# songxf1024/GIMS

Measured on NVIDIA B200. Metric: image_pairs_per_sec_2048kp, higher is better.
Workload: dtype f32

## Files before the change

gims_b200/csrc/gemm_tc.cu:

```cuda
#include "common.cuh"
#include "tc_common.cuh"

namespace gims {

namespace tc {

EncodeTiledFn get_encode_tiled() {
  static EncodeTiledFn fn = nullptr;
  if (fn) return fn;
  void* p = nullptr;
  cudaDriverEntryPointQueryResult qres;
  if (cudaGetDriverEntryPoint("cuTensorMapEncodeTiled", &p, cudaEnableDefault, &qres) != cudaSuccess ||
      qres != cudaDriverEntryPointSuccess)
    return nullptr;
  fn = reinterpret_cast<EncodeTiledFn>(p);
  return fn;
}

int make_tmap_f32_k32(CUtensorMap* out, const float* base, uint64_t rows, uint64_t cols, uint64_t ld, uint32_t box_rows) {
  EncodeTiledFn enc = get_encode_tiled();
  if (!enc) { set_error("cuTensorMapEncodeTiled entry point not available"); return GIMS_ERR_CUDA; }
  cuuint64_t dims[2] = {cols, rows};
  cuuint64_t strides[1] = {ld * sizeof(float)};
  cuuint32_t box[2] = {32, box_rows};
// ... 24 lines not shown
              (unsigned long long)rows, (unsigned long long)cols, (unsigned long long)ld, box_rows);
    return GIMS_ERR_CUDA;
  }
  return GIMS_OK;
}

}

namespace {

using namespace tc;

constexpr int BM = 128, BK = 32;
constexpr int kThreadsTc = 224;
__host__ __device__ constexpr int tc_threads(int prec) { return prec ? kThreadsTc + 128 : kThreadsTc; }

template <int BN, int PREC>
struct TcCfg {
  static constexpr int kBlockK = PREC ? 64 : 32;
  static constexpr int kABytes = BM * kBlockK * 4;
  static constexpr int kWBytes = PREC ? BN * 64 * 2 : BN * BK * 4;
  static constexpr int kStageBytes = kABytes + 2 * kWBytes;
  static constexpr int kStages = PREC ? (BN <= 64 ? 2 : (BN <= 128 ? 3 : 2))
                                      : ((BN <= 64) ? 3 : (BN <= 128 ? 4 : 3));
  static constexpr int kIssuers = 2;
  static constexpr bool kFold = true;
  static constexpr int kMainAcc = 2;
  static constexpr int kCorrAcc = kFold ? 0 : kIssuers;
  static constexpr int kAccCols = (kMainAcc + kCorrAcc) * BN;
  static constexpr int kTmemCols = (BN <= 64) ? 256 : 512;
  static constexpr int kRing = (kTmemCols - kAccCols) / 64 >= 4 ? 4 : 2;
  static constexpr int kRingCol = kAccCols;
  static_assert(kAccCols + kRing * 64 <= kTmemCols, "accumulators + A ring exceed TMEM");
  static constexpr int kBarriers = 2 * kStages + 2 * kRing + 1;
  static constexpr int kBiasOff = (kBarriers * 8 + 16 + 15) & ~15;
  static constexpr int kSmemBytes = kStages * kStageBytes + 1024  + kBiasOff + BN * 4;
};

struct TcArgs {
  int K0, K1;
  const float* bias;
  const float* R; int ldr;
  float* Y; int ldy;
  int N;
  int relu;
  float scale;
  int score;
  Segs segs;
  int tile_end[kMaxSegs];
  int qkv;
  float* qp; void* kp; void* vt; int ldv; int rows_total; int vbase[kMaxSegs];
  unsigned* status;
  const float* wscale_inv;
  int single_chain;
};

__device__ long long* g_gemm_trace = nullptr;

struct TileCoord { int seg, rows, ncols, r0, c0, rbase; };

template <int BN, int MODE, int PREC, typename Ready>
__device__ __forceinline__ void epilogue_tile(const TcArgs& g, const TileCoord& tcd, uint32_t lane_base, int n_main, int n_corr,
                                              int grp, int kGroups, int q, int lane, uint32_t stg, const float* bias_s,
                                              Ready&& ready, long long* trace, bool tr0) {
  using Cfg = TcCfg<BN, PREC>;
  const int seg = tcd.seg, rows = tcd.rows, ncols = tcd.ncols, r0 = tcd.r0, c0 = tcd.c0, rbase = tcd.rbase;
  const float wsc = (PREC && g.wscale_inv) ? *g.wscale_inv : 1.f;
  constexpr int kStgLd = 36;
  const int rl0 = lane >> 3, cj = (lane & 7) * 4;
  const int rfirst = r0 + 32 * q + rl0;
  const int nvalid = rows - rfirst;
  const bool use_r = MODE == 0 && g.R != nullptr;
  const float* rrow = use_r ? g.R + (size_t)(rbase + rfirst) * g.ldr + c0 + cj : nullptr;
  float4 rres[8];
#pragma unroll
  for (int i = 0; i < 8; ++i)
    rres[i] = (use_r && 4 * i < nvalid && c0 + 32 * grp + cj < ncols) ? *reinterpret_cast<const float4*>(rrow + (size_t)(4 * i) * g.ldr + 32 * grp)
                                                           : make_float4(0.f, 0.f, 0.f, 0.f);
  ready();
  if (trace && tr0) trace[3] = clock64();
#pragma unroll 1
  for (int cc = grp; cc < BN / 32; cc += kGroups) {
    uint32_t v[32];
    const uint32_t lane_col = lane_base + (uint32_t)(cc * 32);
    tmem_ld_32x32(lane_col, v);
    tmem_ld_wait();
    for (int a = 1; a < Cfg::kMainAcc + Cfg::kCorrAcc; ++a) {
      if (a < Cfg::kMainAcc ? a >= n_main : a - Cfg::kMainAcc >= n_corr) continue;
      uint32_t w[32];
      tmem_ld_32x32(lane_col + (uint32_t)(a * BN), w);
      tmem_ld_wait();
#pragma unroll
      for (int j = 0; j < 32; ++j) v[j] = __float_as_uint(__uint_as_float(v[j]) + __uint_as_float(w[j]));
    }
    if (PREC) {
#pragma unroll
      for (int j = 0; j < 32; ++j) v[j] = __float_as_uint(__uint_as_float(v[j]) * wsc);
    }
    if (trace && tr0 && cc < 2) trace[56 + 3 * cc] = clock64();
    const int c = c0 + cc * 32;
    if (c >= ncols) continue;
    if (MODE >= 2 && c >= 2 * kD) {
      const int r = r0 + 32 * q + lane;
      if (r < ((g.segs.nmax[seg] + 63) & ~63)) {
        const bool row_ok = r < rows;
        const int cc256 = c & 255;
        const size_t kcol = (size_t)g.vbase[seg] + r;
// ... 291 lines not shown
            hi[j] = __float_as_uint(h); x[j] = __float_as_uint(l);
          }
        }
        mbar_wait(&tfree[slot], ((uint32_t)(kb / Cfg::kRing) & 1u) ^ 1u);
        tcgen05_fence_after();
        if (trace && tr0 && kb < 8) trace[48 + kb] = clock64();
        if (PREC) {
          uint32_t h16[16], l16[16];
#pragma unroll
          for (int j = 0; j < 16; ++j) { h16[j] = hi[j]; l16[j] = x[j]; }
          tmem_st_32x16(lane_base + Cfg::kRingCol + slot * 64 + 16 * grp, h16);
          tmem_st_32x16(lane_base + Cfg::kRingCol + slot * 64 + 32 + 16 * grp, l16);
        } else {
          tmem_st_32x32(lane_base + Cfg::kRingCol + slot * 64, hi);
          tmem_st_32x32(lane_base + Cfg::kRingCol + slot * 64 + 32, x);
        }
        tmem_st_wait();
        tcgen05_fence_before();
        __syncwarp();
        if (lane == 0) mbar_arrive(&conv[slot]);
        if (trace && tr0 && kb < 8) trace[16 + kb] = clock64();
        if (++s == Cfg::kStages) { s = 0; ph ^= 1; }
      }
    }
    if (PREC && g.status && amax >= 32768.f && r0 + t < rows) atomicOr(g.status, GIMS_STATUS_FP16_RANGE);
    {
      const int n_main = nkb < Cfg::kMainAcc ? nkb : Cfg::kMainAcc;
      const int n_corr = nkb < Cfg::kCorrAcc ? nkb : Cfg::kCorrAcc;
      const TileCoord tcd = {seg, rows, ncols, r0, c0, rbase};
      const uint32_t stg = smem_u32(smem) + (uint32_t)((q + 4 * grp) * 32 * 36 * 4);
      epilogue_tile<BN, MODE, PREC>(g, tcd, lane_base, n_main, n_corr, grp, kGroups, q, lane, stg, bias_s,
                                    [&] { mbar_wait(accum_full, 0); tcgen05_fence_after(); }, trace, tr0);
    }
    tcgen05_fence_before();
    if (trace && tr0) trace[4] = clock64();
  }
  __syncthreads();
  if (warp == kWarpMma) {
    tcgen05_fence_after();
    tmem_dealloc<Cfg::kTmemCols>(tmem_base);
  }
  if (trace && threadIdx.x == 0) {
    trace[5] = clock64();
    unsigned long long gt; asm volatile("mov.u64 %0, %%globaltimer;" : "=l"(gt));
    trace[7] = (long long)gt;
  }
}

constexpr int kThreadsP = 480;
struct TcpCfg {
  static constexpr int BN = 128;
  static constexpr int kBlockK = 64;
  static constexpr int kABytes = BM * kBlockK * 4;
  static constexpr int kWBytes = BN * 64 * 2;
  static constexpr int kStageBytes = kABytes + 2 * kWBytes;
  static constexpr int kStages = 3;
  static constexpr int kRing = 2;
  static constexpr int kParkCol = 2 * BN;
  static constexpr int kRingCol = 3 * BN;
  static constexpr int kStgBytes = 4 * 32 * 36 * 4;
  static constexpr int kBarriers = 2 * kStages + 2 * kRing + 4;
  static constexpr int kBiasOff = (kBarriers * 8 + 16 + 15) & ~15;
  static constexpr int kSmemBytes = kStages * kStageBytes + kStgBytes + 1024  + kBiasOff + 2 * BN * 4;
};

template <int MODE, int PLANES>
__global__ void __launch_bounds__(kThreadsP, 1)
k_gemm_tcp(const __grid_constant__ CUtensorMap mapA0, const __grid_constant__ CUtensorMap mapA1,
           const __grid_constant__ CUtensorMap mapWhi, const __grid_constant__ CUtensorMap mapWlo, TcArgs g, int col_tiles,
           int total_work) {
  using Cfg = TcpCfg;
  constexpr int BN = Cfg::BN;
  extern __shared__ uint8_t smem_raw[];
  uint8_t* smem = reinterpret_cast<uint8_t*>((reinterpret_cast<uintptr_t>(smem_raw) + 1023) & ~uintptr_t(1023));
  uint8_t* stg_base = smem + Cfg::kStages * Cfg::kStageBytes;
  uint64_t* bars = reinterpret_cast<uint64_t*>(stg_base + Cfg::kStgBytes);
  uint64_t* full = bars;
  uint64_t* empty = bars + Cfg::kStages;
  uint64_t* conv = bars + 2 * Cfg::kStages;
  uint64_t* tfree = conv + Cfg::kRing;
  uint64_t* accum_full = tfree + Cfg::kRing;
  uint64_t* acc_free = accum_full + 1;
  uint64_t* park_full = acc_free + 1;
  uint64_t* park_free = park_full + 1;
  uint32_t* tmem_slot = reinterpret_cast<uint32_t*>(park_free + 1);
  float* bias_s = reinterpret_cast<float*>(reinterpret_cast<uint8_t*>(bars) + Cfg::kBiasOff);

  const int warp = threadIdx.x >> 5, lane = threadIdx.x & 31;
  constexpr int kWarpTma = 4, kWarpMma = 5, kWarpEpi = 11;
  long long* trace = (blockIdx.x == 0 && lane == 0) ? g_gemm_trace : nullptr;
  if (trace && threadIdx.x == 0) trace[0] = clock64();
#define TCP_TRACE(k) do { if (trace && lt < 4) trace[8 + lt * 8 + (k)] = clock64(); } while (0)
  const int nkb = (g.K0 + g.K1) / Cfg::kBlockK;
  const bool single = g.single_chain != 0;
  const int n_issuers = (nkb >= 2 && !single) ? 2 : 1;

  __shared__ int cnt_s[kMaxSegs];
  if (threadIdx.x < kMaxSegs) cnt_s[threadIdx.x] = (int)threadIdx.x < g.segs.nseg ? seg_count(g.segs, threadIdx.x) : 0;
  auto decode = [&](int w, TileCoord& t, bool from_global = false) -> bool {
    const int rt = w / col_tiles, ct = w - rt * col_tiles;
    int seg = 0, tile = rt;
    if (MODE != 1) {
      while (seg + 1 < g.segs.nseg && rt >= g.tile_end[seg]) ++seg;
      tile = rt - (seg ? g.tile_end[seg - 1] : 0);
    }
    t.seg = seg;
    t.rows = from_global ? seg_count(g.segs, seg) : cnt_s[seg];
    t.ncols = MODE == 1 ? (from_global ? seg_count(g.segs, 1) : cnt_s[1]) : g.N;
    t.r0 = tile * BM; t.c0 = ct * BN;
    t.rbase = g.segs.base[seg];
    return t.r0 < t.rows && t.c0 < t.ncols;
  };
  const int wbase = MODE == 1 ? g.segs.base[1] : 0;

  if (warp == kWarpTma && lane == 0) {
    tma_prefetch_desc(&mapA0);
    if (g.K1) tma_prefetch_desc(&mapA1);
    tma_prefetch_desc(&mapWhi);
    tma_prefetch_desc(&mapWlo);
    for (int s = 0; s < Cfg::kStages; ++s) { mbar_init(&full[s], 1); mbar_init(&empty[s], 1); }
    for (int s = 0; s < Cfg::kRing; ++s) { mbar_init(&conv[s], 8); mbar_init(&tfree[s], 1); }
    mbar_init(accum_full, n_issuers);
    mbar_init(acc_free, 8);
    mbar_init(park_full, 8);
    mbar_init(park_free, 4);
    fence_barrier_init();
  }
  if (warp == kWarpMma) tmem_alloc<512>(tmem_slot);
  tcgen05_fence_before();
  if (warp == kWarpTma) asm volatile("bar.arrive 1, %0;" ::"n"(kThreadsP) : "memory");
  else                  asm volatile("bar.sync 1, %0;" ::"n"(kThreadsP) : "memory");
  tcgen05_fence_after();
  const uint32_t tmem_base = __shfl_sync(0xffffffffu, *tmem_slot, 0);
  auto stage_ptr = [&](int s) { return smem + (size_t)s * Cfg::kStageBytes; };

  if (warp == kWarpTma) {
    if (lane == 0) {
      int s = 0; uint32_t ph = 0;
      for (int w = blockIdx.x; w < total_work; w += gridDim.x) {
        TileCoord t;
        if (!decode(w, t, true)) continue;
        for (int kb = 0; kb < nkb; ++kb) {
          mbar_wait(&empty[s], ph ^ 1);
          uint8_t* st = stage_ptr(s);
          mbar_arrive_expect_tx(&full[s], Cfg::kABytes + PLANES * Cfg::kWBytes);
          const int k = kb * Cfg::kBlockK;
#pragma unroll
          for (int h = 0; h < 2; ++h) {
            const int ka = k + 32 * h;
            if (ka < g.K0) tma_load_2d(st + h * 16384, &mapA0, &full[s], ka, t.rbase + t.r0);
            else           tma_load_2d(st + h * 16384, &mapA1, &full[s], ka - g.K0, t.rbase + t.r0);
          }
          tma_load_2d(st + Cfg::kABytes, &mapWhi, &full[s], k, wbase + t.c0);
          if (PLANES == 2) tma_load_2d(st + Cfg::kABytes + Cfg::kWBytes, &mapWlo, &full[s], k, wbase + t.c0);
          if (++s == Cfg::kStages) { s = 0; ph ^= 1; }
        }
      }
    }
  } else if (warp == kWarpMma || warp == kWarpMma + 1) {
    const int t = __shfl_sync(0xffffffffu, warp - kWarpMma, 0);
    if (lane == 0) {
      constexpr uint32_t idesc = umma_idesc_f16(BM, BN, PLANES == 2 ? 0 : 1);
      const uint64_t d_stage0 = umma_desc_sw128(smem_u32(stage_ptr(0) + Cfg::kABytes));
      const uint32_t acc = tmem_base + t * BN;
      const int kstep = single ? 1 : 2;
      int last = -1;
      if (!(single && t > 0))
        for (int kb = t; kb < nkb; kb += kstep) last = kb;
      int lt = 0;
      for (int w = blockIdx.x; w < total_work; w += gridDim.x) {
        TileCoord tcd;
        if (!decode(w, tcd)) continue;
        if (lt > 0 && last >= 0) { mbar_wait(acc_free, (uint32_t)(lt - 1) & 1u); tcgen05_fence_after(); }
        for (int kb = t; kb < nkb && last >= 0; kb += kstep) {
          const int gk = lt * nkb + kb;
          const int s = gk % Cfg::kStages, slot = gk % Cfg::kRing;
          mbar_wait(&conv[slot], (uint32_t)(gk / Cfg::kRing) & 1u);
          tcgen05_fence_after();
          const uint64_t w_hi = d_stage0 + (uint64_t)((s * Cfg::kStageBytes) >> 4);
          const uint64_t w_lo = w_hi + (Cfg::kWBytes >> 4);
          const uint32_t a_hi = tmem_base + Cfg::kRingCol + slot * 64;
          const uint32_t a_lo = a_hi + 32;
          const uint32_t fresh = kb >= kstep ? 1u : 0u;
          if (t == 0 && kb == 0) TCP_TRACE(7);
#pragma unroll
          for (int ks = 0; ks < 4; ++ks) {
            const uint64_t koff = (ks * 32) >> 4;
            if (PLANES == 2) {
              umma_f16_ts(acc, a_lo + ks * 8, w_hi + koff, idesc, ks ? 1u : fresh);
              umma_f16_ts(acc, a_hi + ks * 8, w_lo + koff, idesc, 1u);
              umma_f16_ts(acc, a_hi + ks * 8, w_hi + koff, idesc, 1u);
            } else {
              umma_f16_ts(acc, a_hi + ks * 8, w_hi + koff, idesc, ks ? 1u : fresh);
            }
          }
          umma_commit(&empty[s]);
          umma_commit(&tfree[slot]);
          if (kb == last) umma_commit(accum_full);
        }
        ++lt;
      }
    }
  } else if (warp < 4 || (warp >= 7 && warp < kWarpEpi)) {
    const int grp = warp >= 7 ? 1 : 0;
    const int q = warp & 3;
    const int t = 32 * q + lane;
    const uint32_t lane_base = tmem_base + ((uint32_t)(32 * q) << 16);
    const int n_main = (nkb < 2 || single) ? 1 : 2;
    auto fold = [&](int f) {
      int lt = f;
      mbar_wait(accum_full, (uint32_t)f & 1u);
      tcgen05_fence_after();
      if (warp == 0) TCP_TRACE(2);
      if (f > 0) { mbar_wait(park_free, (uint32_t)(f - 1) & 1u); tcgen05_fence_after(); }
      if (warp == 0) TCP_TRACE(3);
#pragma unroll
      for (int cc = grp; cc < BN / 32; cc += 2) {
        uint32_t v[32];
        tmem_ld_32x32(lane_base + (uint32_t)(cc * 32), v);
        if (n_main > 1) {
          uint32_t x[32];
          tmem_ld_32x32(lane_base + (uint32_t)(BN + cc * 32), x);
          tmem_ld_wait();
#pragma unroll
          for (int j = 0; j < 32; ++j) v[j] = __float_as_uint(__uint_as_float(v[j]) + __uint_as_float(x[j]));
        } else {
          tmem_ld_wait();
        }
        tmem_st_32x32(lane_base + (uint32_t)(Cfg::kParkCol + cc * 32), v);
      }
      tmem_st_wait();
      tcgen05_fence_before();
      __syncwarp();
      if (lane == 0) { mbar_arrive(acc_free); mbar_arrive(park_full); }
      if (warp == 0) TCP_TRACE(4);
    };
    int lt = 0;
    for (int w = blockIdx.x; w < total_work; w += gridDim.x) {
      TileCoord tcd;
      if (!decode(w, tcd)) continue;
      float amax = 0.f;
      for (int kb = 0; kb < nkb; ++kb) {
        const int gk = lt * nkb + kb;
        const int s = gk % Cfg::kStages, slot = gk % Cfg::kRing;
        mbar_wait(&full[s], (uint32_t)(gk / Cfg::kStages) & 1u);
        if (warp == 0 && kb == 0) TCP_TRACE(0);
        uint32_t hi[16], lo[16];
        const uint4* rowp = reinterpret_cast<const uint4*>(stage_ptr(s) + grp * 16384 + t * 128);
#pragma unroll
        for (int j = 0; j < 8; ++j) {
          const uint4 v = rowp[j ^ (t & 7)];
          const float f0 = __uint_as_float(v.x), f1 = __uint_as_float(v.y), f2 = __uint_as_float(v.z), f3 = __uint_as_float(v.w);
          if (PLANES == 2) {
            amax = fmaxf(amax, fmaxf(fmaxf(fabsf(f0), fabsf(f1)), fmaxf(fabsf(f2), fabsf(f3))));
            split16x2<0>(f0, f1, hi[2 * j], lo[2 * j]);
            split16x2<0>(f2, f3, hi[2 * j + 1], lo[2 * j + 1]);
          } else {
            hi[2 * j] = pack16<1>(f0, f1);
            hi[2 * j + 1] = pack16<1>(f2, f3);
          }
        }
        mbar_wait(&tfree[slot], ((uint32_t)(gk / Cfg::kRing) & 1u) ^ 1u);
        tcgen05_fence_after();
        tmem_st_32x16(lane_base + Cfg::kRingCol + slot * 64 + 16 * grp, hi);
        if (PLANES == 2) tmem_st_32x16(lane_base + Cfg::kRingCol + slot * 64 + 32 + 16 * grp, lo);
        tmem_st_wait();
        tcgen05_fence_before();
        __syncwarp();
        if (lane == 0) mbar_arrive(&conv[slot]);
      }
      if (warp == 0) TCP_TRACE(1);
      if (PLANES == 2 && g.status && amax >= 32768.f && tcd.r0 + t < tcd.rows) atomicOr(g.status, GIMS_STATUS_FP16_RANGE);
      fold(lt);
      ++lt;
    }
  } else {
    const int q = warp & 3;
    const int et = threadIdx.x - kWarpEpi * 32;
    const uint32_t lane_base = tmem_base + ((uint32_t)(32 * q) << 16) + Cfg::kParkCol;
    const uint32_t stg = smem_u32(stg_base) + (uint32_t)((warp - kWarpEpi) * 32 * 36 * 4);
    int lt = 0;
    for (int w = blockIdx.x; w < total_work; w += gridDim.x) {
      TileCoord tcd;
      if (!decode(w, tcd)) continue;
      float* bias_t = bias_s + (lt & 1) * BN;
      bias_t[et] = (g.bias && tcd.c0 + et < g.N) ? g.bias[tcd.c0 + et] : 0.f;
      asm volatile("bar.sync 2, 128;" ::: "memory");
      epilogue_tile<BN, MODE, 1>(g, tcd, lane_base, 1, 0, 0, 1, q, lane, stg, bias_t,
                                 [&] { mbar_wait(park_full, (uint32_t)lt & 1u); tcgen05_fence_after();
                                       if (warp == kWarpEpi) TCP_TRACE(5); }, nullptr, false);
      tcgen05_fence_before();
      __syncwarp();
      if (lane == 0) mbar_arrive(park_free);
      if (warp == kWarpEpi) TCP_TRACE(6);
      ++lt;
    }
  }
#undef TCP_TRACE
  __syncthreads();
  if (warp == kWarpMma) {
    tcgen05_fence_after();
    tmem_dealloc<512>(tmem_base);
  }
  if (trace && threadIdx.x == 0) trace[1] = clock64();
}

__global__ void k_split_planes(const float* __restrict__ x, float* __restrict__ hi, float* __restrict__ lo, size_t n4) {
  size_t i = (size_t)blockIdx.x * blockDim.x + threadIdx.x;
  if (i >= n4) return;
  float4 v = reinterpret_cast<const float4*>(x)[i], h, l;
  tc::split_tf32(v.x, h.x, l.x); tc::split_tf32(v.y, h.y, l.y); tc::split_tf32(v.z, h.z, l.z); tc::split_tf32(v.w, h.w, l.w);
  reinterpret_cast<float4*>(hi)[i] = h;
  reinterpret_cast<float4*>(lo)[i] = l;
}

__global__ void k_split_planes16(const float* __restrict__ x, uint16_t* __restrict__ hi, uint16_t* __restrict__ lo, size_t n4,
                                 unsigned* status) {
  size_t i = (size_t)blockIdx.x * blockDim.x + threadIdx.x;
  if (i >= n4) return;
  const float4 v = reinterpret_cast<const float4*>(x)[i];
  uint2 h, l;
  tc::split16x2<0>(v.x, v.y, h.x, l.x);
  tc::split16x2<0>(v.z, v.w, h.y, l.y);
  reinterpret_cast<uint2*>(hi)[i] = h;
  reinterpret_cast<uint2*>(lo)[i] = l;
  const float m = fmaxf(fmaxf(fabsf(v.x), fabsf(v.y)), fmaxf(fabsf(v.z), fabsf(v.w)));
  if (status && m >= 32768.f && m < 3e38f) atomicOr(status, GIMS_STATUS_FP16_RANGE);
}

__global__ void k_plane_bf16(const float* __restrict__ x, uint16_t* __restrict__ hi, size_t n4) {
  size_t i = (size_t)blockIdx.x * blockDim.x + threadIdx.x;
  if (i >= n4) return;
  const float4 v = reinterpret_cast<const float4*>(x)[i];
  uint2 h;
  h.x = tc::pack16<1>(v.x, v.y);
  h.y = tc::pack16<1>(v.z, v.w);
  reinterpret_cast<uint2*>(hi)[i] = h;
}

template <int BN, int MODE, int PREC = 0>
int launch_tc(const CUtensorMap& a0, const CUtensorMap& a1, const CUtensorMap& whi, const CUtensorMap& wlo,
              const TcArgs& g, int col_tiles, int row_tiles, int prof_class, cudaStream_t st) {
  using Cfg = TcCfg<BN, PREC>;
  GIMS_CUDA_OK(cudaFuncSetAttribute(k_gemm_tc<BN, MODE, PREC>, cudaFuncAttributeMaxDynamicSharedMemorySize, Cfg::kSmemBytes));
  cudaLaunchConfig_t cfg = {};
  cfg.gridDim = dim3(col_tiles, row_tiles);
  cfg.blockDim = dim3(tc_threads(PREC));
  cfg.dynamicSmemBytes = Cfg::kSmemBytes;
  cfg.stream = st;
  cfg.attrs = nullptr;
  cfg.numAttrs = 0;
  ProfScope prof(prof_class, st);
  GIMS_CUDA_OK(cudaLaunchKernelEx(&cfg, k_gemm_tc<BN, MODE, PREC>, a0, a1, whi, wlo, g));
  count_launch();
  return GIMS_OK;
}

int single_chain_knob() {
  static const int on = [] { const char* e = getenv("GIMS_GEMM_SINGLE_CHAIN"); return (e && e[0] == '1') ? 1 : 0; }();
  return on;
}
bool persist_enabled() {
  static const bool on = [] { const char* e = getenv("GIMS_GEMM_PERSIST"); return !(e && e[0] == '0'); }();
  return on;
}
template <int MODE, int PLANES = 2>
int launch_tcp(const CUtensorMap& a0, const CUtensorMap& a1, const CUtensorMap& whi, const CUtensorMap& wlo,
               const TcArgs& g, int col_tiles, int row_tiles, int prof_class, cudaStream_t st) {
  static const int tpc_env = [] { const char* e = getenv("GIMS_GEMM_TPC"); int v = e ? atoi(e) : 2; return v < 1 ? 1 : v; }();
  int dev = 0, sms = 0;
  GIMS_CUDA_OK(cudaGetDevice(&dev));
  GIMS_CUDA_OK(cudaDeviceGetAttribute(&sms, cudaDevAttrMultiProcessorCount, dev));
  const int total = col_tiles * row_tiles;
  const int tpc = (2 * total <= sms) ? 1 : tpc_env;
  int grid = (total + tpc - 1) / tpc;
  if (grid > sms) grid = sms;
  GIMS_CUDA_OK(cudaFuncSetAttribute(k_gemm_tcp<MODE, PLANES>, cudaFuncAttributeMaxDynamicSharedMemorySize, TcpCfg::kSmemBytes));
  cudaLaunchConfig_t cfg = {};
  cfg.gridDim = dim3(grid);
  cfg.blockDim = dim3(kThreadsP);
  cfg.dynamicSmemBytes = TcpCfg::kSmemBytes;
  cfg.stream = st;
  cfg.attrs = nullptr;
  cfg.numAttrs = 0;
  ProfScope prof(prof_class, st);
  GIMS_CUDA_OK(cudaLaunchKernelEx(&cfg, k_gemm_tcp<MODE, PLANES>, a0, a1, whi, wlo, g, col_tiles, total));
  count_launch();
  return GIMS_OK;
}

int pick_bn(int n) {
  static const int forced = [] { const char* e = getenv("GIMS_GEMM_BN"); return e ? atoi(e) : 0; }();
  if (forced == 64 || forced == 128 || forced == 192) return forced;
  if (n >= 768) return 192;
  if (n >= 256) return 128;
  return 64;
}

}

int launch_gemm_tc(const GemmArgs& a, const WPlanes& w, int prec, cudaStream_t st, const QkvPlanes* qkv) {
  int K = a.K0 + a.K1;
  if (prec && (a.K0 % 64 || a.K1 % 64 || !w.h16 || !w.l16 || !w.sinv)) prec = 0;
  if (a.K0 % BK || a.K1 % BK || K == 0 || a.N % 32 || (a.lda0 % 4) || (a.K1 && (a.lda1 % 4)) || !w.hi32 || !w.lo32) {
    set_error("launch_gemm_tc: unsupported shape K0=%d K1=%d N=%d", a.K0, a.K1, a.N);
    return GIMS_ERR_ARG;
  }
  int total_rows = segs_rows(a.segs);
  int bn = pick_bn(a.N);
  if (qkv && (bn != 64 || qkv->fmt >= 0)) bn = 192;
  if (prec) bn = (qkv || (a.N >= 256 && bn != 64)) ? 128 : 64;
  CUtensorMap mA0, mA1, mWh, mWl;
  GIMS_TRY(tc::make_tmap_f32_k32(&mA0, a.A0, total_rows, a.K0, a.lda0, BM));
  if (a.K1) GIMS_TRY(tc::make_tmap_f32_k32(&mA1, a.A1, total_rows, a.K1, a.lda1, BM));
  else mA1 = mA0;
  if (prec) {
    GIMS_TRY(tc::make_tmap_16_k64(&mWh, w.h16, 0, a.N, K, K, bn));
    GIMS_TRY(tc::make_tmap_16_k64(&mWl, w.l16, 0, a.N, K, K, bn));
  } else {
    GIMS_TRY(tc::make_tmap_f32_k32(&mWh, w.hi32, a.N, K, K, bn));
    GIMS_TRY(tc::make_tmap_f32_k32(&mWl, w.lo32, a.N, K, K, bn));
  }
  TcArgs g;
  g.K0 = a.K0; g.K1 = a.K1; g.bias = a.bias; g.R = a.R; g.ldr = a.ldr; g.Y = a.Y; g.ldy = a.ldy; g.N = a.N;
  g.relu = a.relu; g.scale = 1.f; g.score = 0; g.segs = a.segs;
  g.qkv = 0; g.qp = nullptr; g.kp = g.vt = nullptr; g.ldv = 0; g.rows_total = total_rows; g.status = a.status;
  g.wscale_inv = prec ? w.sinv : nullptr;
  g.single_chain = single_chain_knob();
  for (int i = 0; i < kMaxSegs; ++i) g.vbase[i] = 0;
  if (qkv) {
    if (a.N != 3 * kD || !a.bias) { set_error("launch_gemm_tc: qkv mode needs N = 768 and a bias"); return GIMS_ERR_ARG; }
    g.qkv = 1; g.qp = qkv->qp; g.kp = qkv->kp; g.vt = qkv->vt; g.ldv = qkv->ldv;
    for (int i = 0; i < kMaxSegs; ++i) g.vbase[i] = qkv->vbase[i];
    if (qkv->status) g.status = qkv->status;
  }
  int tiles = 0;
  for (int i = 0; i < a.segs.nseg; ++i) { tiles += cdiv(a.segs.nmax[i], BM); g.tile_end[i] = tiles; }
  if (tiles == 0) return GIMS_OK;
  int ct = cdiv(a.N, bn);
  if (qkv) {
    if (qkv->fmt >= 0 && !((qkv->fmt == 0 && qkv->planes == 2) || (qkv->fmt == 1 && qkv->planes == 1))) {
      set_error("launch_gemm_tc: unsupported 16-bit plane format");
      return GIMS_ERR_ARG;
    }
    if (prec && persist_enabled()) {
      if (qkv->fmt == 0) return launch_tcp<3>(mA0, mA1, mWh, mWl, g, ct, tiles, GIMS_PROF_GEMM, st);
      if (qkv->fmt == 1) return launch_tcp<4>(mA0, mA1, mWh, mWl, g, ct, tiles, GIMS_PROF_GEMM, st);
      return launch_tcp<2>(mA0, mA1, mWh, mWl, g, ct, tiles, GIMS_PROF_GEMM, st);
    }
    if (prec) {
      if (qkv->fmt == 0) return launch_tc<128, 3, 1>(mA0, mA1, mWh, mWl, g, ct, tiles, GIMS_PROF_GEMM, st);
      if (qkv->fmt == 1) return launch_tc<128, 4, 1>(mA0, mA1, mWh, mWl, g, ct, tiles, GIMS_PROF_GEMM, st);
      return launch_tc<128, 2, 1>(mA0, mA1, mWh, mWl, g, ct, tiles, GIMS_PROF_GEMM, st);
    }
    if (qkv->fmt == 0) return launch_tc<192, 3>(mA0, mA1, mWh, mWl, g, ct, tiles, GIMS_PROF_GEMM, st);
    if (qkv->fmt == 1) return launch_tc<192, 4>(mA0, mA1, mWh, mWl, g, ct, tiles, GIMS_PROF_GEMM, st);
    if (bn == 64) return launch_tc<64, 2>(mA0, mA1, mWh, mWl, g, ct, tiles, GIMS_PROF_GEMM, st);
    return launch_tc<192, 2>(mA0, mA1, mWh, mWl, g, ct, tiles, GIMS_PROF_GEMM, st);
  }
  if (prec) {
    if (bn == 128 && persist_enabled()) return launch_tcp<0>(mA0, mA1, mWh, mWl, g, ct, tiles, GIMS_PROF_GEMM, st);
    if (bn == 128) return launch_tc<128, 0, 1>(mA0, mA1, mWh, mWl, g, ct, tiles, GIMS_PROF_GEMM, st);
    return launch_tc<64, 0, 1>(mA0, mA1, mWh, mWl, g, ct, tiles, GIMS_PROF_GEMM, st);
  }
  switch (bn) {
    case 192: return launch_tc<192, 0>(mA0, mA1, mWh, mWl, g, ct, tiles, GIMS_PROF_GEMM, st);
    case 128: return launch_tc<128, 0>(mA0, mA1, mWh, mWl, g, ct, tiles, GIMS_PROF_GEMM, st);
    default:  return launch_tc<64, 0>(mA0, mA1, mWh, mWl, g, ct, tiles, GIMS_PROF_GEMM, st);
  }
}

int set_gemm_trace(long long* dev_buf) {
  GIMS_CUDA_OK(cudaMemcpyToSymbol(g_gemm_trace, &dev_buf, sizeof(dev_buf)));
  return GIMS_OK;
}

int launch_split_planes(const float* x, float* hi, float* lo, size_t n, cudaStream_t st) {
  size_t n4 = n / 4;
  k_split_planes<<<(unsigned)((n4 + 255) / 256), 256, 0, st>>>(x, hi, lo, n4);
  GIMS_LAUNCH_OK();
  return GIMS_OK;
}

int launch_score_gemm_tc(const float* mdesc, int n0_max, int n1_max, const int* n_dev, float* planes, float* couplings,
                         int prec, unsigned* status, cudaStream_t st) {
  size_t rows = (size_t)n0_max + n1_max;
  constexpr int bn = 128;
  CUtensorMap mA, mWh, mWl;
  GIMS_TRY(tc::make_tmap_f32_k32(&mA, mdesc, rows, kD, kD, BM));
  if (prec == 2) {
    uint16_t* hi = reinterpret_cast<uint16_t*>(planes);
    k_plane_bf16<<<(unsigned)((rows * kD / 4 + 255) / 256), 256, 0, st>>>(mdesc, hi, rows * kD / 4);
    GIMS_LAUNCH_OK();
    GIMS_TRY(tc::make_tmap_16_k64(&mWh, hi, 1, rows, kD, kD, bn));
    mWl = mWh;
  } else if (prec) {
    uint16_t* hi = reinterpret_cast<uint16_t*>(planes);
    uint16_t* lo = hi + rows * kD;
    k_split_planes16<<<(unsigned)((rows * kD / 4 + 255) / 256), 256, 0, st>>>(mdesc, hi, lo, rows * kD / 4, status);
    GIMS_LAUNCH_OK();
    GIMS_TRY(tc::make_tmap_16_k64(&mWh, hi, 0, rows, kD, kD, bn));
    GIMS_TRY(tc::make_tmap_16_k64(&mWl, lo, 0, rows, kD, kD, bn));
  } else {
    float* hi = planes;
    float* lo = planes + rows * kD;
    GIMS_TRY(launch_split_planes(mdesc, hi, lo, rows * kD, st));
    GIMS_TRY(tc::make_tmap_f32_k32(&mWh, hi, rows, kD, kD, bn));
    GIMS_TRY(tc::make_tmap_f32_k32(&mWl, lo, rows, kD, kD, bn));
  }
  TcArgs g;
  g.K0 = kD; g.K1 = 0; g.bias = nullptr; g.R = nullptr; g.ldr = 0; g.Y = couplings; g.ldy = coup_ld(n1_max); g.N = n1_max;
  g.relu = 0; g.scale = 0.0625f; g.score = 1;
  g.qkv = 0; g.qp = nullptr; g.kp = g.vt = nullptr; g.ldv = 0; g.rows_total = (int)rows; g.status = status;
  g.wscale_inv = nullptr;
  g.single_chain = single_chain_knob();
  for (int i = 0; i < kMaxSegs; ++i) { g.vbase[i] = 0; g.tile_end[i] = 0; }
  g.segs = two_segs(n0_max, n1_max, n_dev);
  g.tile_end[0] = cdiv(n0_max, BM);
  if (prec == 2) return launch_tcp<1, 1>(mA, mA, mWh, mWl, g, cdiv(n1_max, bn), g.tile_end[0], GIMS_PROF_SCORE, st);
  if (prec && persist_enabled()) return launch_tcp<1>(mA, mA, mWh, mWl, g, cdiv(n1_max, bn), g.tile_end[0], GIMS_PROF_SCORE, st);
  if (prec) return launch_tc<bn, 1, 1>(mA, mA, mWh, mWl, g, cdiv(n1_max, bn), g.tile_end[0], GIMS_PROF_SCORE, st);
  return launch_tc<bn, 1>(mA, mA, mWh, mWl, g, cdiv(n1_max, bn), g.tile_end[0], GIMS_PROF_SCORE, st);
}

}
```

gims_b200/csrc/tc_common.cuh:

```cuda
#pragma once
#include <cuda.h>
#include <cuda_runtime.h>
#include <stdint.h>

namespace gims {
namespace tc {

__device__ __forceinline__ uint32_t smem_u32(const void* p) { return (uint32_t)__cvta_generic_to_shared(p); }

__device__ __forceinline__ void mbar_init(uint64_t* bar, uint32_t count) {
  asm volatile("mbarrier.init.shared::cta.b64 [%0], %1;" ::"r"(smem_u32(bar)), "r"(count) : "memory");
}
__device__ __forceinline__ void fence_barrier_init() { asm volatile("fence.mbarrier_init.release.cluster;" ::: "memory"); }
__device__ __forceinline__ void mbar_arrive(uint64_t* bar) {
  asm volatile("mbarrier.arrive.shared::cta.b64 _, [%0];" ::"r"(smem_u32(bar)) : "memory");
}
__device__ __forceinline__ void mbar_arrive_expect_tx(uint64_t* bar, uint32_t bytes) {
  asm volatile("mbarrier.arrive.expect_tx.shared::cta.b64 _, [%0], %1;" ::"r"(smem_u32(bar)), "r"(bytes) : "memory");
}
static __device__ unsigned g_tc_timeout_flag;
static __device__ unsigned g_tc_timeout_info[4];
__device__ __forceinline__ bool mbar_try_wait(uint32_t addr, uint32_t parity) {
  uint32_t ok;
  asm volatile(
// ... 102 lines not shown
}
__device__ __forceinline__ void tmem_st_wait() { asm volatile("tcgen05.wait::st.sync.aligned;" ::: "memory"); }

__device__ __forceinline__ void umma_tf32_ts(uint32_t tmem_d, uint32_t tmem_a, uint64_t desc_b, uint32_t idesc,
                                             uint32_t accumulate) {
  asm volatile(
      "{\n\t.reg .pred p;\n\t"
      "setp.ne.b32 p, %4, 0;\n\t"
      "tcgen05.mma.cta_group::1.kind::tf32 [%0], [%1], %2, %3, p;\n\t}" ::"r"(tmem_d),
      "r"(tmem_a), "l"(desc_b), "r"(idesc), "r"(accumulate)
      : "memory");
}
__host__ __device__ constexpr uint32_t umma_idesc_f16(int m, int n, int fmt) {
  return (1u << 4) | ((uint32_t)fmt << 7) | ((uint32_t)fmt << 10) | ((uint32_t)(n >> 3) << 17) | ((uint32_t)(m >> 4) << 24);
}
__device__ __forceinline__ void umma_f16_ts(uint32_t tmem_d, uint32_t tmem_a, uint64_t desc_b, uint32_t idesc,
                                            uint32_t accumulate) {
  asm volatile(
      "{\n\t.reg .pred p;\n\t"
      "setp.ne.b32 p, %4, 0;\n\t"
      "tcgen05.mma.cta_group::1.kind::f16 [%0], [%1], %2, %3, p;\n\t}" ::"r"(tmem_d),
      "r"(tmem_a), "l"(desc_b), "r"(idesc), "r"(accumulate)
      : "memory");
}
template <int FMT>
__device__ __forceinline__ uint32_t pack16(float lo, float hi) {
  uint32_t d;
  if (FMT == 0) asm("cvt.rn.f16x2.f32 %0, %1, %2;" : "=r"(d) : "f"(hi), "f"(lo));
  else          asm("cvt.rn.bf16x2.f32 %0, %1, %2;" : "=r"(d) : "f"(hi), "f"(lo));
  return d;
}
template <int FMT>
__device__ __forceinline__ void unpack16(uint32_t d, float& lo, float& hi) {
  if (FMT == 0) {
    asm("{\n\t.reg .f16 l, h;\n\tmov.b32 {l, h}, %2;\n\tcvt.f32.f16 %0, l;\n\tcvt.f32.f16 %1, h;\n\t}" : "=f"(lo), "=f"(hi) : "r"(d));
  } else {
    lo = __uint_as_float(d << 16);
    hi = __uint_as_float(d & 0xffff0000u);
  }
}
template <int FMT>
__device__ __forceinline__ void split16x2(float x0, float x1, uint32_t& hi, uint32_t& lo) {
  hi = pack16<FMT>(x0, x1);
  float h0, h1;
  unpack16<FMT>(hi, h0, h1);
  lo = pack16<FMT>(x0 - h0, x1 - h1);
}

__device__ __forceinline__ void umma_commit(uint64_t* bar) {
  asm volatile("tcgen05.commit.cta_group::1.mbarrier::arrive::one.shared::cluster.b64 [%0];" ::"r"(smem_u32(bar))
               : "memory");
}

__device__ __forceinline__ void split_tf32(float x, float& hi, float& lo) {
  const uint32_t h = (__float_as_uint(x) + 0x1000u) & 0xffffe000u;
  hi = __uint_as_float(h);
  lo = x - hi;
}

typedef CUresult (*EncodeTiledFn)(CUtensorMap*, CUtensorMapDataType, cuuint32_t, void*, const cuuint64_t*,
                                  const cuuint64_t*, const cuuint32_t*, const cuuint32_t*, CUtensorMapInterleave,
                                  CUtensorMapSwizzle, CUtensorMapL2promotion, CUtensorMapFloatOOBfill);
EncodeTiledFn get_encode_tiled();
int make_tmap_f32_k32(CUtensorMap* out, const float* base, uint64_t rows, uint64_t cols, uint64_t ld, uint32_t box_rows);
int make_tmap_16_k64(CUtensorMap* out, const void* base, int fmt, uint64_t rows, uint64_t cols, uint64_t ld, uint32_t box_rows);

}
}
```

Measured before the change: 664.8.

## Run persistent pair GEMM as 2-CTA cluster with cta_group::2 UMMA

Converts the persistent pair-plane GEMM kernel into a two-CTA cluster. Each pair of CTAs covers two row tiles with one M=256 tcgen05 MMA issued by rank 0. Each CTA loads half of the W tile, which halves per-CTA weight traffic and shared memory per stage, and the freed space buys a fourth pipeline stage. Barriers, TMEM allocation and commits become cluster-scoped, the single-chain debug knob is dropped, and drain loops are added before teardown. This adds cross-CTA synchronisation and complexity, and halves the number of independent work units when there are few tiles.

```diff
diff --git a/gims_b200/csrc/gemm_tc.cu b/gims_b200/csrc/gemm_tc.cu
--- a/gims_b200/csrc/gemm_tc.cu
+++ b/gims_b200/csrc/gemm_tc.cu
@@ -100,7 +100,6 @@
   float* qp; void* kp; void* vt; int ldv; int rows_total; int vbase[kMaxSegs];
   unsigned* status;
   const float* wscale_inv;
-  int single_chain;
 };
 
 __device__ long long* g_gemm_trace = nullptr;
@@ -498,9 +497,9 @@
   static constexpr int BN = 128;
   static constexpr int kBlockK = 64;
   static constexpr int kABytes = BM * kBlockK * 4;
-  static constexpr int kWBytes = BN * 64 * 2;
-  static constexpr int kStageBytes = kABytes + 2 * kWBytes;
-  static constexpr int kStages = 3;
+  static constexpr int kWHalfBytes = (BN / 2) * 64 * 2;
+  static constexpr int kStageBytes = kABytes + 2 * kWHalfBytes;
+  static constexpr int kStages = 4;
   static constexpr int kRing = 2;
   static constexpr int kParkCol = 2 * BN;
   static constexpr int kRingCol = 3 * BN;
@@ -508,6 +507,7 @@
   static constexpr int kBarriers = 2 * kStages + 2 * kRing + 4;
   static constexpr int kBiasOff = (kBarriers * 8 + 16 + 15) & ~15;
   static constexpr int kSmemBytes = kStages * kStageBytes + kStgBytes + 1024  + kBiasOff + 2 * BN * 4;
+  static_assert(kSmemBytes <= 227 * 1024, "pair kernel exceeds the shared memory of an SM");
 };
 
 template <int MODE, int PLANES>
@@ -534,28 +534,35 @@
 
   const int warp = threadIdx.x >> 5, lane = threadIdx.x & 31;
   constexpr int kWarpTma = 4, kWarpMma = 5, kWarpEpi = 11;
+  const uint32_t rank = cluster_ctarank();
+  const int cluster = blockIdx.x >> 1, nclusters = gridDim.x >> 1;
   long long* trace = (blockIdx.x == 0 && lane == 0) ? g_gemm_trace : nullptr;
   if (trace && threadIdx.x == 0) trace[0] = clock64();
 #define TCP_TRACE(k) do { if (trace && lt < 4) trace[8 + lt * 8 + (k)] = clock64(); } while (0)
   const int nkb = (g.K0 + g.K1) / Cfg::kBlockK;
-  const bool single = g.single_chain != 0;
-  const int n_issuers = (nkb >= 2 && !single) ? 2 : 1;
+  const int n_issuers = nkb >= 2 ? 2 : 1;
 
   __shared__ int cnt_s[kMaxSegs];
   if (threadIdx.x < kMaxSegs) cnt_s[threadIdx.x] = (int)threadIdx.x < g.segs.nseg ? seg_count(g.segs, threadIdx.x) : 0;
-  auto decode = [&](int w, TileCoord& t, bool from_global = false) -> bool {
-    const int rt = w / col_tiles, ct = w - rt * col_tiles;
+  auto tile_of = [&](int rt, int ct, TileCoord& t) -> bool {
     int seg = 0, tile = rt;
     if (MODE != 1) {
       while (seg + 1 < g.segs.nseg && rt >= g.tile_end[seg]) ++seg;
       tile = rt - (seg ? g.tile_end[seg - 1] : 0);
     }
     t.seg = seg;
-    t.rows = from_global ? seg_count(g.segs, seg) : cnt_s[seg];
-    t.ncols = MODE == 1 ? (from_global ? seg_count(g.segs, 1) : cnt_s[1]) : g.N;
+    t.rows = cnt_s[seg];
+    t.ncols = MODE == 1 ? cnt_s[1] : g.N;
     t.r0 = tile * BM; t.c0 = ct * BN;
     t.rbase = g.segs.base[seg];
-    return t.r0 < t.rows && t.c0 < t.ncols;
+    return t.r0 < t.rows;
+  };
+  auto decode = [&](int w, TileCoord& t, bool& live) -> bool {
+    const int rp = w / col_tiles, ct = w - rp * col_tiles;
+    TileCoord o;
+    const bool l0 = tile_of(2 * rp, ct, rank ? o : t), l1 = tile_of(2 * rp + 1, ct, rank ? t : o);
+    live = rank ? l1 : l0;
+    return (l0 || l1) && t.c0 < t.ncols;
   };
   const int wbase = MODE == 1 ? g.segs.base[1] : 0;
 
@@ -563,19 +570,18 @@
     tma_prefetch_desc(&mapA0);
     if (g.K1) tma_prefetch_desc(&mapA1);
     tma_prefetch_desc(&mapWhi);
-    tma_prefetch_desc(&mapWlo);
+    if (PLANES == 2) tma_prefetch_desc(&mapWlo);
     for (int s = 0; s < Cfg::kStages; ++s) { mbar_init(&full[s], 1); mbar_init(&empty[s], 1); }
-    for (int s = 0; s < Cfg::kRing; ++s) { mbar_init(&conv[s], 8); mbar_init(&tfree[s], 1); }
+    for (int s = 0; s < Cfg::kRing; ++s) { mbar_init(&conv[s], 16); mbar_init(&tfree[s], 1); }
     mbar_init(accum_full, n_issuers);
-    mbar_init(acc_free, 8);
+    mbar_init(acc_free, 16);
     mbar_init(park_full, 8);
     mbar_init(park_free, 4);
     fence_barrier_init();
   }
-  if (warp == kWarpMma) tmem_alloc<512>(tmem_slot);
+  if (warp == kWarpMma) tmem_alloc_pair<512>(tmem_slot);
   tcgen05_fence_before();
-  if (warp == kWarpTma) asm volatile("bar.arrive 1, %0;" ::"n"(kThreadsP) : "memory");
-  else                  asm volatile("bar.sync 1, %0;" ::"n"(kThreadsP) : "memory");
+  cluster_sync();
   tcgen05_fence_after();
   const uint32_t tmem_base = __shfl_sync(0xffffffffu, *tmem_slot, 0);
   auto stage_ptr = [&](int s) { return smem + (size_t)s * Cfg::kStageBytes; };
@@ -583,13 +589,14 @@
   if (warp == kWarpTma) {
     if (lane == 0) {
       int s = 0; uint32_t ph = 0;
-      for (int w = blockIdx.x; w < total_work; w += gridDim.x) {
-        TileCoord t;
-        if (!decode(w, t, true)) continue;
+      constexpr uint32_t kWBytes = 2 * PLANES * Cfg::kWHalfBytes;
+      for (int w = cluster; w < total_work; w += nclusters) {
+        TileCoord t; bool live;
+        if (!decode(w, t, live)) continue;
         for (int kb = 0; kb < nkb; ++kb) {
           mbar_wait(&empty[s], ph ^ 1);
           uint8_t* st = stage_ptr(s);
-          mbar_arrive_expect_tx(&full[s], Cfg::kABytes + PLANES * Cfg::kWBytes);
+          mbar_arrive_expect_tx(&full[s], Cfg::kABytes + (rank ? 0u : kWBytes));
           const int k = kb * Cfg::kBlockK;
 #pragma unroll
           for (int h = 0; h < 2; ++h) {
@@ -597,52 +604,57 @@
             if (ka < g.K0) tma_load_2d(st + h * 16384, &mapA0, &full[s], ka, t.rbase + t.r0);
             else           tma_load_2d(st + h * 16384, &mapA1, &full[s], ka - g.K0, t.rbase + t.r0);
           }
-          tma_load_2d(st + Cfg::kABytes, &mapWhi, &full[s], k, wbase + t.c0);
-          if (PLANES == 2) tma_load_2d(st + Cfg::kABytes + Cfg::kWBytes, &mapWlo, &full[s], k, wbase + t.c0);
+          const uint32_t wbar = mapa_shared(&full[s], 0);
+          const int wrow = wbase + t.c0 + (int)rank * (BN / 2);
+          tma_load_2d_pair(st + Cfg::kABytes, &mapWhi, wbar, k, wrow);
+          if (PLANES == 2) tma_load_2d_pair(st + Cfg::kABytes + Cfg::kWHalfBytes, &mapWlo, wbar, k, wrow);
           if (++s == Cfg::kStages) { s = 0; ph ^= 1; }
         }
+      }
+      for (int i = 0; i < Cfg::kStages; ++i) {
+        mbar_wait(&empty[s], ph ^ 1);
+        if (++s == Cfg::kStages) { s = 0; ph ^= 1; }
       }
     }
   } else if (warp == kWarpMma || warp == kWarpMma + 1) {
     const int t = __shfl_sync(0xffffffffu, warp - kWarpMma, 0);
-    if (lane == 0) {
-      constexpr uint32_t idesc = umma_idesc_f16(BM, BN, PLANES == 2 ? 0 : 1);
+    if (rank == 0 && lane == 0 && t < n_issuers) {
+      constexpr uint32_t idesc = umma_idesc_f16(2 * BM, BN, PLANES == 2 ? 0 : 1);
       const uint64_t d_stage0 = umma_desc_sw128(smem_u32(stage_ptr(0) + Cfg::kABytes));
       const uint32_t acc = tmem_base + t * BN;
-      const int kstep = single ? 1 : 2;
       int last = -1;
-      if (!(single && t > 0))
-        for (int kb = t; kb < nkb; kb += kstep) last = kb;
+      for (int kb = t; kb < nkb; kb += 2) last = kb;
       int lt = 0;
-      for (int w = blockIdx.x; w < total_work; w += gridDim.x) {
-        TileCoord tcd;
-        if (!decode(w, tcd)) continue;
-        if (lt > 0 && last >= 0) { mbar_wait(acc_free, (uint32_t)(lt - 1) & 1u); tcgen05_fence_after(); }
-        for (int kb = t; kb < nkb && last >= 0; kb += kstep) {
+      for (int w = cluster; w < total_work; w += nclusters) {
+        TileCoord tcd; bool live;
+        if (!decode(w, tcd, live)) continue;
+        if (lt > 0) { mbar_wait(acc_free, (uint32_t)(lt - 1) & 1u); tcgen05_fence_after(); }
+        for (int kb = t; kb < nkb; kb += 2) {
           const int gk = lt * nkb + kb;
           const int s = gk % Cfg::kStages, slot = gk % Cfg::kRing;
+          mbar_wait(&full[s], (uint32_t)(gk / Cfg::kStages) & 1u);
           mbar_wait(&conv[slot], (uint32_t)(gk / Cfg::kRing) & 1u);
           tcgen05_fence_after();
           const uint64_t w_hi = d_stage0 + (uint64_t)((s * Cfg::kStageBytes) >> 4);
-          const uint64_t w_lo = w_hi + (Cfg::kWBytes >> 4);
+          const uint64_t w_lo = w_hi + (Cfg::kWHalfBytes >> 4);
           const uint32_t a_hi = tmem_base + Cfg::kRingCol + slot * 64;
           const uint32_t a_lo = a_hi + 32;
-          const uint32_t fresh = kb >= kstep ? 1u : 0u;
+          const uint32_t fresh = kb >= 2 ? 1u : 0u;
           if (t == 0 && kb == 0) TCP_TRACE(7);
 #pragma unroll
           for (int ks = 0; ks < 4; ++ks) {
             const uint64_t koff = (ks * 32) >> 4;
             if (PLANES == 2) {
-              umma_f16_ts(acc, a_lo + ks * 8, w_hi + koff, idesc, ks ? 1u : fresh);
-              umma_f16_ts(acc, a_hi + ks * 8, w_lo + koff, idesc, 1u);
-              umma_f16_ts(acc, a_hi + ks * 8, w_hi + koff, idesc, 1u);
+              umma_f16_ts_pair(acc, a_lo + ks * 8, w_hi + koff, idesc, ks ? 1u : fresh);
+              umma_f16_ts_pair(acc, a_hi + ks * 8, w_lo + koff, idesc, 1u);
+              umma_f16_ts_pair(acc, a_hi + ks * 8, w_hi + koff, idesc, 1u);
             } else {
-              umma_f16_ts(acc, a_hi + ks * 8, w_hi + koff, idesc, ks ? 1u : fresh);
+              umma_f16_ts_pair(acc, a_hi + ks * 8, w_hi + koff, idesc, ks ? 1u : fresh);
             }
           }
-          umma_commit(&empty[s]);
-          umma_commit(&tfree[slot]);
-          if (kb == last) umma_commit(accum_full);
+          umma_commit_pair(&empty[s]);
+          umma_commit_pair(&tfree[slot]);
+          if (kb == last) umma_commit_pair(accum_full);
         }
         ++lt;
       }
@@ -652,7 +664,7 @@
     const int q = warp & 3;
     const int t = 32 * q + lane;
     const uint32_t lane_base = tmem_base + ((uint32_t)(32 * q) << 16);
-    const int n_main = (nkb < 2 || single) ? 1 : 2;
+    const int n_main = nkb < 2 ? 1 : 2;
     auto fold = [&](int f) {
       int lt = f;
       mbar_wait(accum_full, (uint32_t)f & 1u);
@@ -678,13 +690,13 @@
       tmem_st_wait();
       tcgen05_fence_before();
       __syncwarp();
-      if (lane == 0) { mbar_arrive(acc_free); mbar_arrive(park_full); }
+      if (lane == 0) { mbar_arrive_remote(mapa_shared(acc_free, 0)); mbar_arrive(park_full); }
       if (warp == 0) TCP_TRACE(4);
     };
     int lt = 0;
-    for (int w = blockIdx.x; w < total_work; w += gridDim.x) {
-      TileCoord tcd;
-      if (!decode(w, tcd)) continue;
+    for (int w = cluster; w < total_work; w += nclusters) {
+      TileCoord tcd; bool live;
+      if (!decode(w, tcd, live)) continue;
       float amax = 0.f;
       for (int kb = 0; kb < nkb; ++kb) {
         const int gk = lt * nkb + kb;
@@ -713,12 +725,16 @@
         tmem_st_wait();
         tcgen05_fence_before();
         __syncwarp();
-        if (lane == 0) mbar_arrive(&conv[slot]);
+        if (lane == 0) mbar_arrive_remote(mapa_shared(&conv[slot], 0));
       }
       if (warp == 0) TCP_TRACE(1);
       if (PLANES == 2 && g.status && amax >= 32768.f && tcd.r0 + t < tcd.rows) atomicOr(g.status, GIMS_STATUS_FP16_RANGE);
       fold(lt);
       ++lt;
+    }
+    for (int i = 0; i < Cfg::kRing; ++i) {
+      const int gk = lt * nkb + i;
+      mbar_wait(&tfree[gk % Cfg::kRing], ((uint32_t)(gk / Cfg::kRing) & 1u) ^ 1u);
     }
   } else {
     const int q = warp & 3;
@@ -726,15 +742,18 @@
     const uint32_t lane_base = tmem_base + ((uint32_t)(32 * q) << 16) + Cfg::kParkCol;
     const uint32_t stg = smem_u32(stg_base) + (uint32_t)((warp - kWarpEpi) * 32 * 36 * 4);
     int lt = 0;
-    for (int w = blockIdx.x; w < total_work; w += gridDim.x) {
-      TileCoord tcd;
-      if (!decode(w, tcd)) continue;
-      float* bias_t = bias_s + (lt & 1) * BN;
-      bias_t[et] = (g.bias && tcd.c0 + et < g.N) ? g.bias[tcd.c0 + et] : 0.f;
-      asm volatile("bar.sync 2, 128;" ::: "memory");
-      epilogue_tile<BN, MODE, 1>(g, tcd, lane_base, 1, 0, 0, 1, q, lane, stg, bias_t,
-                                 [&] { mbar_wait(park_full, (uint32_t)lt & 1u); tcgen05_fence_after();
-                                       if (warp == kWarpEpi) TCP_TRACE(5); }, nullptr, false);
+    for (int w = cluster; w < total_work; w += nclusters) {
+      TileCoord tcd; bool live;
+      if (!decode(w, tcd, live)) continue;
+      auto ready = [&] { mbar_wait(park_full, (uint32_t)lt & 1u); tcgen05_fence_after(); if (warp == kWarpEpi) TCP_TRACE(5); };
+      if (live) {
+        float* bias_t = bias_s + (lt & 1) * BN;
+        bias_t[et] = (g.bias && tcd.c0 + et < g.N) ? g.bias[tcd.c0 + et] : 0.f;
+        asm volatile("bar.sync 2, 128;" ::: "memory");
+        epilogue_tile<BN, MODE, 1>(g, tcd, lane_base, 1, 0, 0, 1, q, lane, stg, bias_t, ready, nullptr, false);
+      } else {
+        ready();
+      }
       tcgen05_fence_before();
       __syncwarp();
       if (lane == 0) mbar_arrive(park_free);
@@ -743,12 +762,13 @@
     }
   }
 #undef TCP_TRACE
-  __syncthreads();
+  tcgen05_fence_before();
+  cluster_sync();
   if (warp == kWarpMma) {
     tcgen05_fence_after();
-    tmem_dealloc<512>(tmem_base);
-  }
-  if (trace && threadIdx.x == 0) trace[1] = clock64();
+    tmem_dealloc_pair<512>(*tmem_slot);
+  }
+  if (blockIdx.x == 0 && threadIdx.x == 0 && g_gemm_trace) g_gemm_trace[1] = clock64();
 }
 
 __global__ void k_split_planes(const float* __restrict__ x, float* __restrict__ hi, float* __restrict__ lo, size_t n4) {
@@ -802,10 +822,6 @@
   return GIMS_OK;
 }
 
-int single_chain_knob() {
-  static const int on = [] { const char* e = getenv("GIMS_GEMM_SINGLE_CHAIN"); return (e && e[0] == '1') ? 1 : 0; }();
-  return on;
-}
 bool persist_enabled() {
   static const bool on = [] { const char* e = getenv("GIMS_GEMM_PERSIST"); return !(e && e[0] == '0'); }();
   return on;
@@ -817,18 +833,22 @@
   int dev = 0, sms = 0;
   GIMS_CUDA_OK(cudaGetDevice(&dev));
   GIMS_CUDA_OK(cudaDeviceGetAttribute(&sms, cudaDevAttrMultiProcessorCount, dev));
-  const int total = col_tiles * row_tiles;
-  const int tpc = (2 * total <= sms) ? 1 : tpc_env;
-  int grid = (total + tpc - 1) / tpc;
-  if (grid > sms) grid = sms;
+  const int max_clusters = sms / 2;
+  const int total = col_tiles * ((row_tiles + 1) / 2);
+  const int ipc = (2 * total <= max_clusters) ? 1 : tpc_env;
+  int clusters = (total + ipc - 1) / ipc;
+  if (clusters > max_clusters) clusters = max_clusters;
   GIMS_CUDA_OK(cudaFuncSetAttribute(k_gemm_tcp<MODE, PLANES>, cudaFuncAttributeMaxDynamicSharedMemorySize, TcpCfg::kSmemBytes));
+  cudaLaunchAttribute attr[1];
+  attr[0].id = cudaLaunchAttributeClusterDimension;
+  attr[0].val.clusterDim.x = 2; attr[0].val.clusterDim.y = 1; attr[0].val.clusterDim.z = 1;
   cudaLaunchConfig_t cfg = {};
-  cfg.gridDim = dim3(grid);
+  cfg.gridDim = dim3(2 * clusters);
   cfg.blockDim = dim3(kThreadsP);
   cfg.dynamicSmemBytes = TcpCfg::kSmemBytes;
   cfg.stream = st;
-  cfg.attrs = nullptr;
-  cfg.numAttrs = 0;
+  cfg.attrs = attr;
+  cfg.numAttrs = 1;
   ProfScope prof(prof_class, st);
   GIMS_CUDA_OK(cudaLaunchKernelEx(&cfg, k_gemm_tcp<MODE, PLANES>, a0, a1, whi, wlo, g, col_tiles, total));
   count_launch();
@@ -860,9 +880,10 @@
   GIMS_TRY(tc::make_tmap_f32_k32(&mA0, a.A0, total_rows, a.K0, a.lda0, BM));
   if (a.K1) GIMS_TRY(tc::make_tmap_f32_k32(&mA1, a.A1, total_rows, a.K1, a.lda1, BM));
   else mA1 = mA0;
+  const bool pair = prec && bn == 128 && persist_enabled();
   if (prec) {
-    GIMS_TRY(tc::make_tmap_16_k64(&mWh, w.h16, 0, a.N, K, K, bn));
-    GIMS_TRY(tc::make_tmap_16_k64(&mWl, w.l16, 0, a.N, K, K, bn));
+    GIMS_TRY(tc::make_tmap_16_k64(&mWh, w.h16, 0, a.N, K, K, pair ? bn / 2 : bn));
+    GIMS_TRY(tc::make_tmap_16_k64(&mWl, w.l16, 0, a.N, K, K, pair ? bn / 2 : bn));
   } else {
     GIMS_TRY(tc::make_tmap_f32_k32(&mWh, w.hi32, a.N, K, K, bn));
     GIMS_TRY(tc::make_tmap_f32_k32(&mWl, w.lo32, a.N, K, K, bn));
@@ -872,7 +893,6 @@
   g.relu = a.relu; g.scale = 1.f; g.score = 0; g.segs = a.segs;
   g.qkv = 0; g.qp = nullptr; g.kp = g.vt = nullptr; g.ldv = 0; g.rows_total = total_rows; g.status = a.status;
   g.wscale_inv = prec ? w.sinv : nullptr;
-  g.single_chain = single_chain_knob();
   for (int i = 0; i < kMaxSegs; ++i) g.vbase[i] = 0;
   if (qkv) {
     if (a.N != 3 * kD || !a.bias) { set_error("launch_gemm_tc: qkv mode needs N = 768 and a bias"); return GIMS_ERR_ARG; }
@@ -889,7 +909,7 @@
       set_error("launch_gemm_tc: unsupported 16-bit plane format");
       return GIMS_ERR_ARG;
     }
-    if (prec && persist_enabled()) {
+    if (pair) {
       if (qkv->fmt == 0) return launch_tcp<3>(mA0, mA1, mWh, mWl, g, ct, tiles, GIMS_PROF_GEMM, st);
       if (qkv->fmt == 1) return launch_tcp<4>(mA0, mA1, mWh, mWl, g, ct, tiles, GIMS_PROF_GEMM, st);
       return launch_tcp<2>(mA0, mA1, mWh, mWl, g, ct, tiles, GIMS_PROF_GEMM, st);
@@ -905,7 +925,7 @@
     return launch_tc<192, 2>(mA0, mA1, mWh, mWl, g, ct, tiles, GIMS_PROF_GEMM, st);
   }
   if (prec) {
-    if (bn == 128 && persist_enabled()) return launch_tcp<0>(mA0, mA1, mWh, mWl, g, ct, tiles, GIMS_PROF_GEMM, st);
+    if (pair) return launch_tcp<0>(mA0, mA1, mWh, mWl, g, ct, tiles, GIMS_PROF_GEMM, st);
     if (bn == 128) return launch_tc<128, 0, 1>(mA0, mA1, mWh, mWl, g, ct, tiles, GIMS_PROF_GEMM, st);
     return launch_tc<64, 0, 1>(mA0, mA1, mWh, mWl, g, ct, tiles, GIMS_PROF_GEMM, st);
   }
@@ -933,20 +953,21 @@
   size_t rows = (size_t)n0_max + n1_max;
   constexpr int bn = 128;
   CUtensorMap mA, mWh, mWl;
+  const bool pair = prec == 2 || (prec && persist_enabled());
   GIMS_TRY(tc::make_tmap_f32_k32(&mA, mdesc, rows, kD, kD, BM));
   if (prec == 2) {
     uint16_t* hi = reinterpret_cast<uint16_t*>(planes);
     k_plane_bf16<<<(unsigned)((rows * kD / 4 + 255) / 256), 256, 0, st>>>(mdesc, hi, rows * kD / 4);
     GIMS_LAUNCH_OK();
-    GIMS_TRY(tc::make_tmap_16_k64(&mWh, hi, 1, rows, kD, kD, bn));
+    GIMS_TRY(tc::make_tmap_16_k64(&mWh, hi, 1, rows, kD, kD, bn / 2));
     mWl = mWh;
   } else if (prec) {
     uint16_t* hi = reinterpret_cast<uint16_t*>(planes);
     uint16_t* lo = hi + rows * kD;
     k_split_planes16<<<(unsigned)((rows * kD / 4 + 255) / 256), 256, 0, st>>>(mdesc, hi, lo, rows * kD / 4, status);
     GIMS_LAUNCH_OK();
-    GIMS_TRY(tc::make_tmap_16_k64(&mWh, hi, 0, rows, kD, kD, bn));
-    GIMS_TRY(tc::make_tmap_16_k64(&mWl, lo, 0, rows, kD, kD, bn));
+    GIMS_TRY(tc::make_tmap_16_k64(&mWh, hi, 0, rows, kD, kD, pair ? bn / 2 : bn));
+    GIMS_TRY(tc::make_tmap_16_k64(&mWl, lo, 0, rows, kD, kD, pair ? bn / 2 : bn));
   } else {
     float* hi = planes;
     float* lo = planes + rows * kD;
@@ -959,12 +980,11 @@
   g.relu = 0; g.scale = 0.0625f; g.score = 1;
   g.qkv = 0; g.qp = nullptr; g.kp = g.vt = nullptr; g.ldv = 0; g.rows_total = (int)rows; g.status = status;
   g.wscale_inv = nullptr;
-  g.single_chain = single_chain_knob();
   for (int i = 0; i < kMaxSegs; ++i) { g.vbase[i] = 0; g.tile_end[i] = 0; }
   g.segs = two_segs(n0_max, n1_max, n_dev);
   g.tile_end[0] = cdiv(n0_max, BM);
   if (prec == 2) return launch_tcp<1, 1>(mA, mA, mWh, mWl, g, cdiv(n1_max, bn), g.tile_end[0], GIMS_PROF_SCORE, st);
-  if (prec && persist_enabled()) return launch_tcp<1>(mA, mA, mWh, mWl, g, cdiv(n1_max, bn), g.tile_end[0], GIMS_PROF_SCORE, st);
+  if (pair) return launch_tcp<1>(mA, mA, mWh, mWl, g, cdiv(n1_max, bn), g.tile_end[0], GIMS_PROF_SCORE, st);
   if (prec) return launch_tc<bn, 1, 1>(mA, mA, mWh, mWl, g, cdiv(n1_max, bn), g.tile_end[0], GIMS_PROF_SCORE, st);
   return launch_tc<bn, 1>(mA, mA, mWh, mWl, g, cdiv(n1_max, bn), g.tile_end[0], GIMS_PROF_SCORE, st);
 }
diff --git a/gims_b200/csrc/tc_common.cuh b/gims_b200/csrc/tc_common.cuh
--- a/gims_b200/csrc/tc_common.cuh
+++ b/gims_b200/csrc/tc_common.cuh
@@ -178,6 +178,56 @@
                : "memory");
 }
 
+__device__ __forceinline__ uint32_t cluster_ctarank() {
+  uint32_t r;
+  asm volatile("mov.u32 %0, %%cluster_ctarank;" : "=r"(r));
+  return r;
+}
+__device__ __forceinline__ uint32_t mapa_shared(const void* p, uint32_t rank) {
+  uint32_t r;
+  asm volatile("mapa.shared::cluster.u32 %0, %1, %2;" : "=r"(r) : "r"(smem_u32(p)), "r"(rank));
+  return r;
+}
+__device__ __forceinline__ void mbar_arrive_remote(uint32_t cluster_addr) {
+  asm volatile("mbarrier.arrive.shared::cluster.b64 _, [%0];" ::"r"(cluster_addr) : "memory");
+}
+__device__ __forceinline__ void cluster_sync() {
+  asm volatile("barrier.cluster.arrive.release;\n\tbarrier.cluster.wait.acquire;" ::: "memory");
+}
+__device__ __forceinline__ void tma_load_2d_pair(void* smem_dst, const CUtensorMap* m, uint32_t bar_cluster_addr, int c0, int c1) {
+  asm volatile(
+      "cp.async.bulk.tensor.2d.cta_group::2.shared::cluster.global.mbarrier::complete_tx::bytes [%0], [%1, {%3, %4}], [%2];" ::"r"(
+          smem_u32(smem_dst)),
+      "l"(reinterpret_cast<uint64_t>(m)), "r"(bar_cluster_addr), "r"(c0), "r"(c1)
+      : "memory");
+}
+template <int COLS>
+__device__ __forceinline__ void tmem_alloc_pair(uint32_t* smem_result) {
+  static_assert(COLS == 32 || COLS == 64 || COLS == 128 || COLS == 256 || COLS == 512, "TMEM columns: power of 2 >= 32");
+  asm volatile("tcgen05.alloc.cta_group::2.sync.aligned.shared::cta.b32 [%0], %1;" ::"r"(smem_u32(smem_result)), "n"(COLS)
+               : "memory");
+  asm volatile("tcgen05.relinquish_alloc_permit.cta_group::2.sync.aligned;" ::: "memory");
+}
+template <int COLS>
+__device__ __forceinline__ void tmem_dealloc_pair(uint32_t taddr) {
+  asm volatile("tcgen05.dealloc.cta_group::2.sync.aligned.b32 %0, %1;" ::"r"(taddr), "n"(COLS) : "memory");
+}
+__device__ __forceinline__ void umma_f16_ts_pair(uint32_t tmem_d, uint32_t tmem_a, uint64_t desc_b, uint32_t idesc,
+                                                 uint32_t accumulate) {
+  asm volatile(
+      "{\n\t.reg .pred p;\n\t"
+      "setp.ne.b32 p, %4, 0;\n\t"
+      "tcgen05.mma.cta_group::2.kind::f16 [%0], [%1], %2, %3, p;\n\t}" ::"r"(tmem_d),
+      "r"(tmem_a), "l"(desc_b), "r"(idesc), "r"(accumulate)
+      : "memory");
+}
+__device__ __forceinline__ void umma_commit_pair(uint64_t* bar) {
+  asm volatile("tcgen05.commit.cta_group::2.mbarrier::arrive::one.shared::cluster.multicast::cluster.b64 [%0], %1;" ::"r"(
+                   smem_u32(bar)),
+               "h"((uint16_t)3)
+               : "memory");
+}
+
 __device__ __forceinline__ void split_tf32(float x, float& hi, float& lo) {
   const uint32_t h = (__float_as_uint(x) + 0x1000u) & 0xffffe000u;
   hi = __uint_as_float(h);
```

Result: slower. 656.0 (median of 6 runs) (-1.3%).
